# afriesen/rdis

Measured on AMD Instinct MI355X. Metric: subspace-solver iters/sec (all components), ladybug BA, higher is better.
Workload: dtype f64

## Files before the change

### rdis_amd/csrc/solver_pipe.hpp

```cpp
#pragma once
#include "solver_coop.hpp"

namespace rdis_hip {

constexpr int PIPE_NBUF = 32;
constexpr int PIPE_DEPTH = 3;
constexpr int PIPE_ENT = 512;
constexpr int PIPE_MAILS = 4;
constexpr int PIPE_THREADS = 256;
constexpr int PIPE_CTRL = 2;
constexpr int PIPE_LANES = PIPE_THREADS - 64 * PIPE_CTRL;
constexpr int PIPE_QUIT = 0x7FFFFFFF;
static_assert(PIPE_NBUF >= 5 * PIPE_DEPTH + 4 && (PIPE_NBUF & (PIPE_NBUF - 1)) == 0, "ring too short for the run-ahead");

struct PipeState {
    alignas(32) unsigned long long granule[2][PIPE_NBUF][PIPE_ENT][2];
    unsigned int abort_flag;
    unsigned int pad[15];
};
static_assert(sizeof(PipeState) <= sizeof(CoopState), "PipeState must fit the exchange state the host allocates");

struct alignas(16) PipeMail {
    int kind, flags;
    int e;
    int pad0;
    double a, b;
    double g_a, g_b, g_x, g_dx, g_ax, g_bx, g_cx;
    int g_need_first, g_known;
    double g_w, g_v, g_dw, g_dv, g_d, g_e, g_uu;
    int g_ph, pad1;
};
static_assert(sizeof(PipeMail) == 160, "mail layout");
constexpr int PIPE_RES = 4;
static_assert(PIPE_RES > PIPE_DEPTH, "result ring");
constexpr int PIPE_RECS = 8;
struct PipeShared {
    PipeMail mail[PIPE_MAILS];
    alignas(8) int seq;
    int verified;
    int pred_seq;
    int rec_slot[PIPE_RECS];
    double rec_val[PIPE_RECS];
    int cmd, cmd_delay;
    int res_slot[PIPE_RES];
    double res[PIPE_RES][3];
    int bar_done;
    int pub[PIPE_LANES / 64];
    int dead;
    int status, rolled_back, iter;
    int fin;
    long long nfeval, ngeval;
    double fret, finit;
    CgdMachine mach;
};
typedef __attribute__((address_space(3))) int lds_i32;
typedef __attribute__((address_space(3))) double lds_f64;
__device__ __forceinline__ int lds_int(const int& x) { return *(const volatile lds_i32*)&x; }
__device__ __forceinline__ void lds_set(int& x, int v) { *(volatile lds_i32*)&x = v; }
typedef __attribute__((address_space(3))) long long lds_i64;
__device__ __forceinline__ long long lds_int_pair(const int& x) { return *(const volatile lds_i64*)&x; }
__device__ __forceinline__ double lds_f64_get(const double& x) { return *(const volatile lds_f64*)&x; }
__device__ __forceinline__ void lds_f64_set(double& x, double v) { *(volatile lds_f64*)&x = v; }

struct PipeSync {
    PipeState* st;
    int tid, nwg, wg, nw;
    int poll_delay;
    int e;
    int rearmed;
    bool dead;
#ifdef RDIS_COOP_TIMING
    long long tm[COOP_TM];
#endif
    __device__ void tick(int slot, long long dt) {
#ifdef RDIS_COOP_TIMING
        tm[slot] += dt;
#endif
    }
    __device__ gu64* gran(int ex, int k, int w) const { return (gu64*)&st->granule[k >> 1][ex & (PIPE_NBUF - 1)][w][k & 1]; }
    __device__ u64x2 load_pair(int ex, int k, int w) const {
        u64x2 r;
        const gu64* p = gran(ex, k, w);
        asm volatile("global_load_dwordx4 %0, %1, off sc1" : "=v"(r) : "v"(p) : "memory");
        return r;
    }
    __device__ void store_pair(int ex, int k, int w, unsigned long long a, unsigned long long b) const {
        u64x2 t; t.x = a; t.y = b;
        gu64* p = gran(ex, k, w);
        asm volatile("global_store_dwordx4 %0, %1, off sc1" : : "v"(p), "v"(t) : "memory");
    }

    template <int N, int NMAX>
    __device__ void publish(int ex, double (&v)[N], int* pub) {
#pragma unroll
        for (int k = 0; k < N; ++k) v[k] = k < N - NMAX ? wave_sum(v[k]) : wave_max(v[k]);
        asm volatile("s_waitcnt vmcnt(0)" ::: "memory");
        if ((tid & 63) == 0) {
            const int ent = wg * nw + (tid >> 6) - PIPE_CTRL;
#pragma unroll
            for (int k = 0; k + 1 < N; k += 2) store_pair(ex, k, ent, GridSync::bits_of(v[k]), GridSync::bits_of(v[k + 1]));
            if constexpr (N & 1) GridSync::publish(gran(ex, N - 1, ent), v[N - 1]);
            lds_set(pub[(tid >> 6) - PIPE_CTRL], ex);
        }
    }

    template <int N, int NMAX>
    __device__ bool sweep(int ex, double (&v)[N], int delay, const int& cmd, int cmd_mine, const int* pub) {
        const int lane = tid & 63;
        const int nent = nwg * nw;
        double acc[N];
#pragma unroll
        for (int k = 0; k < N; ++k) acc[k] = 0.0;
        unsigned spins = 0;
        bool ok = !dead;
        const int per = (nent + 63) >> 6;
        constexpr int CH = 8;
        const long long tq0 = coop_clock();
        {
            bool waited = false;
            for (;;) {
                int lo = lds_int(pub[0]);
#pragma unroll
                for (int w = 1; w < PIPE_LANES / 64; ++w) { const int t = lds_int(pub[w]); lo = t < lo ? t : lo; }
                if (lo >= ex || dead) break;
                if (lds_int(cmd) != cmd_mine) return false;
                waited = true;
                if (++spins > COOP_SPIN_LIMIT) break;
                __builtin_amdgcn_s_sleep(1);
            }
            spins = 0;
            if (waited) { tick(26, coop_clock() - tq0); tick(27, 1); }
            if (waited) for (int d = 0; d < delay; d += 8) __builtin_amdgcn_s_sleep(8);
        }
        const long long tq1 = coop_clock();
        for (int j0 = 0; j0 < per && ok; j0 += CH) {
            unsigned long long val[CH][N];
#pragma unroll
            for (int j = 0; j < CH; ++j)
#pragma unroll
                for (int k = 0; k < N; ++k) val[j][k] = COOP_SENTINEL;
            for (;;) {
                tick(6, 1);
                constexpr int NP = N / 2;
                u64x2 pr[CH][NP > 0 ? NP : 1];
#pragma unroll
                for (int j = 0; j < CH; ++j) {
                    const int ww = lane + ((j0 + j) << 6);
                    const int wc = ww < nent ? ww : 0;
#pragma unroll
                    for (int k = 0; k + 1 < N; k += 2) {
                        pr[j][k / 2].x = val[j][k]; pr[j][k / 2].y = val[j][k + 1];
                        if (val[j][k] == COOP_SENTINEL || val[j][k + 1] == COOP_SENTINEL) pr[j][k / 2] = load_pair(ex, k, wc);
                    }
                    if constexpr (N & 1) {
                        if (val[j][N - 1] == COOP_SENTINEL)
                            val[j][N - 1] = __hip_atomic_load(gran(ex, N - 1, wc), __ATOMIC_RELAXED, __HIP_MEMORY_SCOPE_AGENT);
                    }
                }
                if constexpr (NP > 0) {
#pragma unroll
                    for (int j = 0; j < CH; ++j)
#pragma unroll
                        for (int q = 0; q < NP; ++q) asm volatile("" : "+v"(pr[j][q]));
                    asm volatile("s_waitcnt vmcnt(0)" ::: "memory");
#pragma unroll
                    for (int j = 0; j < CH; ++j)
#pragma unroll
                        for (int q = 0; q < NP; ++q) {
                            asm volatile("" : "+v"(pr[j][q]));
                            val[j][2 * q] = pr[j][q].x; val[j][2 * q + 1] = pr[j][q].y;
                        }
                }
                bool here = true;
#pragma unroll
                for (int j = 0; j < CH; ++j)
#pragma unroll
                    for (int k = 0; k < N; ++k) here = here && val[j][k] != COOP_SENTINEL;
                if (__all(here)) break;
                if (lds_int(cmd) != cmd_mine) return false;
                ++spins;
                if (spins > COOP_SPIN_LIMIT ||
                    ((spins & 255u) == 0u &&
                     __hip_atomic_load((gu32*)&st->abort_flag, __ATOMIC_RELAXED, __HIP_MEMORY_SCOPE_AGENT) != 0u)) {
                    if (lane == 0) __hip_atomic_store((gu32*)&st->abort_flag, 1u, __ATOMIC_RELAXED, __HIP_MEMORY_SCOPE_AGENT);
                    ok = false;
                    break;
                }
                __builtin_amdgcn_s_sleep(1);
            }
#pragma unroll
            for (int j = 0; j < CH; ++j) {
                if (lane + ((j0 + j) << 6) < nent) {
#pragma unroll
                    for (int k = 0; k < N; ++k) {
                        const double x = __longlong_as_double(val[j][k]);
                        if (k < N - NMAX) acc[k] += x; else acc[k] = fmax(acc[k], x);
                    }
                }
            }
        }
        if (!__all(ok)) dead = true;
        const long long tq2 = coop_clock();
#pragma unroll
        for (int k = 0; k < N; ++k) v[k] = k < N - NMAX ? wave_sum(acc[k]) : wave_max(acc[k]);
        tick(5, 1); tick(28, tq2 - tq1); tick(29, coop_clock() - tq2);
        return true;
    }
    __device__ void rearm_behind(int ex) {
        const int upto = ex - PIPE_DEPTH - 1;
        if ((tid & 63) < nw) {
            const int ent = wg * nw + (tid & 63);
            for (int x = rearmed + 1; x <= upto; ++x) {
#pragma unroll
                for (int k = 0; k < COOP_KP; k += 2) store_pair(x, k, ent, COOP_SENTINEL, COOP_SENTINEL);
            }
        }
        if (upto > rearmed) rearmed = upto;
    }

    __device__ void barrier(PipeShared& S) {
        double z[1] = {0.0};
        publish<1, 0>(e, z, S.pub);
        while (lds_int(S.bar_done) < e) __builtin_amdgcn_s_sleep(1);
        ++e;
        if (lds_int(S.dead) != 0) dead = true;
    }
};

struct PipeEnv {
    const ProblemView& P;
    const PlanView& L;
    const CoopArgs& A;
    PipeShared& S;
    int n, m, f0, c0;
    int gt, tid;
    PipeSync X;
    double* tr;
    int trn, lm_count;
    bool has_fac;
    int fid;
    int gpos[12];
    double base[12], dirv[12], lov[12], hiv[12];
    double ox, oy;
    VarState lv, wv;

    __device__ void trace(int tag, double a, double b, double c) {
        if (tr != nullptr && X.wg == 0 && tid == 0) {
            if (trn < L.trace_cap) { double* r = tr + 4ll * trn; r[0] = (double)tag; r[1] = a; r[2] = b; r[3] = c; }
            ++trn;
        }
    }

    template <bool SLOPE>
    __device__ void eval_line(double a, double& f, double& s) {
        double fj = 0.0, sj = 0.0;
        if (has_fac) {
            double v[12];
            {
#pragma clang fp contract(off)
#pragma unroll
                for (int k = 0; k < 12; ++k) {
                    const double t = a * dirv[k];
                    v[k] = clampd(base[k] + t, lov[k], hiv[k]);
                }
            }
            if constexpr (SLOPE) {
                double g[12];
                fj = ba_eval_grad(v, ox, oy, g);
                double acc = 0.0;
#pragma unroll
                for (int k = 0; k < 12; ++k) acc = __builtin_fma(g[k], dirv[k], acc);
                sj = acc;
            } else {
                fj = ba_eval(v, ox, oy);
            }
        }
        f = fj; s = sj;
    }
    __device__ void load_base(const double* vec) {
        if (has_fac) {
            const int c = P.cam[fid], q = P.pt[fid];
            const int* sl = A.slot_li + 12ll * gt;
#pragma unroll
            for (int k = 0; k < 12; ++k) {
                const int v = k < 9 ? c + k : q + (k - 9);
                const int li = sl[k];
                if (li >= 0) { base[k] = vec[li]; lov[k] = P.lo[v]; hiv[k] = P.hi[v]; }
                else { base[k] = P.x[v]; lov[k] = -__builtin_inf(); hiv[k] = __builtin_inf(); }
                dirv[k] = 0.0;
            }
        }
    }
    __device__ void var_init(VarState& V, int li) {
        V.li = li;
        V.p = V.xi = V.g = V.h = V.xinit = 0.0; V.lo = V.hi = 0.0;
        if (li >= 0) {
            const int vid = L.free_vid[f0 + li];
            V.p = L.xstart[f0 + li]; V.xinit = V.p;
            V.lo = P.lo[vid]; V.hi = P.hi[vid];
        }
    }
    __device__ void init_vectors() {
        var_init(lv, gt >= 0 ? A.lane_var[gt] : -1);
        var_init(wv, gt >= 0 ? A.wave_var[gt >> 6] : -1);
        load_base(L.xstart + f0);
    }
    __device__ void gradient_to_xi() {
        const long long tg0 = coop_clock();
        if (has_fac) {
            double v[12], g[12];
#pragma unroll
            for (int k = 0; k < 12; ++k) v[k] = clampd(base[k], lov[k], hiv[k]);
            ba_eval_grad(v, ox, oy, g);
#pragma unroll
            for (int k = 0; k < 12; ++k)
                if (gpos[k] >= 0) store_f64<true>(L.gfac + gpos[k], g[k]);
        }
        const long long tg1 = coop_clock();
        X.barrier(S);
        const long long tg2 = coop_clock();
        const int* vp = L.v2s_ptr + f0;
        if (lv.li >= 0) lv.xi = run_sum_ordered<true, 32>(L.gfac, vp[lv.li], vp[lv.li + 1]);
        if (wv.li >= 0) wv.xi = wave_sum(run_sum_strided<true>(L.gfac, vp[wv.li], vp[wv.li + 1], tid & 63));
        X.tick(3, tg1 - tg0); X.tick(18, tg2 - tg1); X.tick(30, coop_clock() - tg2); X.tick(31, 1);
    }
    __device__ void publish_xi() {
        if (lv.li >= 0) store_f64<true>(A.xi_glob + lv.li, lv.xi);
        if (wv.li >= 0 && (tid & 63) == 0) store_f64<true>(A.xi_glob + wv.li, wv.xi);
        X.barrier(S);
    }
    __device__ void cg_start() {
        { const double t = -lv.xi; lv.g = t; lv.h = t; lv.xi = t; }
        { const double t = -wv.xi; wv.g = t; wv.h = t; wv.xi = t; }
        publish_xi();
    }
    template <bool FROM_GH>
    __device__ void line_begin(double gam) {
        if (has_fac) {
            const int* sl = A.slot_li + 12ll * gt;
            int li[12];
#pragma unroll
            for (int k = 0; k < 12; ++k) li[k] = sl[k];
            double d[12];
            if constexpr (FROM_GH) {
                const double* gb = L.ws + 5ll * f0;
#pragma unroll
                for (int k = 0; k < 12; ++k) d[k] = load_f64<true>(gb + (li[k] >= 0 ? li[k] : 0));
                {
#pragma clang fp contract(off)
#pragma unroll
                    for (int k = 0; k < 12; ++k) d[k] = d[k] + gam * dirv[k];
                }
            } else {
#pragma unroll
                for (int k = 0; k < 12; ++k) d[k] = load_f64<true>(A.xi_glob + (li[k] >= 0 ? li[k] : 0));
            }
#pragma unroll
            for (int k = 0; k < 12; ++k) dirv[k] = li[k] >= 0 ? d[k] : 0.0;
        }
        if (L.vdump != nullptr && lm_count < L.dump_iters) {
            double* d = L.vdump + 2ll * L.dump_iters * f0 + 2ll * lm_count * n;
            if (lv.li >= 0) { d[lv.li] = lv.p; d[n + lv.li] = lv.xi; }
            if (wv.li >= 0 && (tid & 63) == 0) { d[wv.li] = wv.p; d[n + wv.li] = wv.xi; }
        }
        ++lm_count;
    }
    __device__ void line_end(double amin) {
#pragma clang fp contract(off)
        { const double t = lv.xi * amin; lv.xi = t; lv.p = lv.p + t; }
        { const double t = wv.xi * amin; wv.xi = t; wv.p = wv.p + t; }
        if (has_fac) {
#pragma unroll
            for (int k = 0; k < 12; ++k) { const double t = dirv[k] * amin; base[k] = base[k] + t; }
        }
    }
    __device__ void cg_reduce_publish(double fp) {
        {
            double* gb = L.ws + 5ll * f0;
            if (lv.li >= 0) store_f64<true>(gb + lv.li, -lv.xi);
            if (wv.li >= 0 && (tid & 63) == 0) store_f64<true>(gb + wv.li, -wv.xi);
        }
        double a = 0.0, b = 0.0, t = 0.0;
        {
#pragma clang fp contract(off)
            const double den = fmax(fabs(fp), 1.0);
            if (lv.li >= 0) {
                t = fabs(lv.xi) * fmax(fabs(lv.p), 1.0) / den;
                a = lv.g * lv.g;
                b = (lv.xi + lv.g) * lv.xi;
            }
            if (wv.li >= 0 && (tid & 63) == 0) {
                t = fmax(t, fabs(wv.xi) * fmax(fabs(wv.p), 1.0) / den);
                a = a + wv.g * wv.g;
                b = b + (wv.xi + wv.g) * wv.xi;
            }
        }
        double v[3] = {a, b, t};
        X.publish<3, 1>(X.e, v, S.pub);
        ++X.e;
    }
    __device__ void cg_update(double gam) {
#pragma clang fp contract(off)
        { const double gn = -lv.xi; const double hn = gn + gam * lv.h; lv.g = gn; lv.h = hn; lv.xi = hn; }
        { const double gn = -wv.xi; const double hn = gn + gam * wv.h; wv.g = gn; wv.h = hn; wv.xi = hn; }
    }
    __device__ void write_back(const VarState& V, bool restore, bool writer) {
        if (V.li >= 0 && writer) {
            const double xf = clampd(restore ? V.xinit : V.p, V.lo, V.hi);
            P.x[L.free_vid[f0 + V.li]] = xf;
            L.xout[f0 + V.li] = xf;
        }
    }
};

__device__ __forceinline__ int pipe_slot_owner(int i) {
    return (i == 0 || i == 2 || i == 3 || i == 18 || (i >= 9 && i <= 11) || i == 30 || i == 31) ? 2 : (i == 1 || (i >= 4 && i <= 6) || (i >= 26 && i <= 29)) ? 1 : 0;
}

__device__ __forceinline__ void pipe_post(PipeShared& S, int seq, int kind, int flags, int e, double a, double b, bool writer) {
    if (writer) {
        PipeMail* m = &S.mail[seq & (PIPE_MAILS - 1)];
        m->kind = kind; m->flags = flags; m->e = e; m->pad0 = 0; m->a = a; m->b = b;
        asm volatile("" ::: "memory");
        lds_set(S.seq, seq);
    }
}
__device__ __forceinline__ void pipe_post_predictor(PipeShared& S, int seq, const Predictor& G, bool writer) {
    if (writer) {
        PipeMail* m = &S.mail[seq & (PIPE_MAILS - 1)];
        m->g_ph = G.ph; m->g_need_first = G.need_first ? 1 : 0; m->g_known = G.known ? 1 : 0; m->pad1 = 0;
        m->g_a = G.a; m->g_b = G.b; m->g_x = G.x; m->g_dx = G.dx; m->g_ax = G.ax; m->g_bx = G.bx; m->g_cx = G.cx;
        m->g_w = G.w; m->g_v = G.v; m->g_dw = G.dw; m->g_dv = G.dv; m->g_d = G.d; m->g_e = G.e; m->g_uu = G.uu;
        asm volatile("" ::: "memory");
        lds_set(S.pred_seq, seq);
    }
}
__device__ __forceinline__ void pipe_command(PipeShared& S, int ex, int n, int delay, bool writer) {
    if (writer) { lds_set(S.cmd_delay, delay); lds_set(S.cmd, (ex << 2) | n); }
}
template <int N>
__device__ __forceinline__ void pipe_result(PipeShared& S, int ex, double (&v)[N], bool& dead) {
    while (lds_int(S.res_slot[ex & (PIPE_RES - 1)]) != ex) __builtin_amdgcn_s_sleep(1);
    asm volatile("" ::: "memory");
#pragma unroll
    for (int k = 0; k < N; ++k) v[k] = uniform(lds_f64_get(S.res[ex & (PIPE_RES - 1)][k]));
    if (lds_int(S.dead) != 0) dead = true;
}
__device__ __forceinline__ void pipe_ctrl_barrier(PipeSync& X, PipeShared& S, bool writer) {
    double z[1];
    pipe_command(S, X.e, 1, X.poll_delay, writer);
    pipe_result(S, X.e, z, X.dead);
    if (writer) lds_set(S.bar_done, X.e);
    ++X.e;
}

__device__ __forceinline__ void pipe_stepper(PipeEnv& E, PipeShared& S, int maxiters, double ftol) {
    CgdMachine& M = S.mach;
    const bool writer = E.tid == 0;
    if (writer) M.init(maxiters, ftol);
    int e_last = 0;
    bool chain_live = false;
    int next_free = 0;
    bool swapped = true;
    double r0 = 0.0, r1 = 0.0, r2 = 0.0;
    int seq = 0;
    bool guessed = false;
    double gval = 0.0;
    int ahead_slot = -1;
    double ahead0 = 0.0, ahead1 = 0.0;
    auto read_chain = [&]() {
        guessed = false; gval = 0.0; ahead_slot = -1; ahead0 = ahead1 = 0.0;
        if (chain_live) {
            const int z = e_last + 1;
            int rec = lds_int(S.rec_slot[z & (PIPE_RECS - 1)]);
            ahead_slot = lds_int(S.res_slot[z & (PIPE_RES - 1)]);
            ahead0 = lds_f64_get(S.res[z & (PIPE_RES - 1)][0]);
            ahead1 = lds_f64_get(S.res[z & (PIPE_RES - 1)][1]);
            while ((rec >> 1) != z) { __builtin_amdgcn_s_sleep(1); rec = lds_int(S.rec_slot[z & (PIPE_RECS - 1)]); }
            guessed = (rec & 1) != 0;
            gval = uniform(lds_f64_get(S.rec_val[z & (PIPE_RECS - 1)]));
        }
    };
    auto await_fd = [&](int e, bool hit) {
        double v[2];
        const long long tw0 = coop_clock();
        if (hit && __builtin_amdgcn_readfirstlane(ahead_slot) == e) {
            v[0] = uniform(ahead0); v[1] = uniform(ahead1);
            if (lds_int(S.dead) != 0) E.X.dead = true;
        } else {
            pipe_result(S, e, v, E.X.dead);
        }
        if (hit) { E.X.tick(20, coop_clock() - tw0); E.X.tick(16, 1); }
        else { E.X.tick(21, coop_clock() - tw0); E.X.tick(17, 1); }
        r0 = v[0]; r1 = v[1];
        e_last = e;
        chain_live = true;
        next_free = e_last + PIPE_DEPTH + 1;
    };
    for (;;) {
        long long ts0 = coop_clock();
        read_chain();
        bool stepped = false;
        if (__builtin_amdgcn_readfirstlane(lds_int(M.st)) == CgdMachine::S_DB_EVAL) {
            BrentHot s = M.brent();
            opaque(s.a); opaque(s.b); opaque(s.x); opaque(s.w); opaque(s.v); opaque(s.fx); opaque(s.fw); opaque(s.fv);
            opaque(s.dx); opaque(s.dw); opaque(s.dv); opaque(s.d); opaque(s.e); opaque(s.uu);
            HotPre P;
            CgdMachine::hot_pre(s, P);
            for (;;) {
                asm volatile("; PIPE_STEP_BEGIN");
                BrentHot n;
                double un;
                const bool take = CgdMachine::hot_post(s, P, r0, r1, n, un);
                if (__builtin_amdgcn_readfirstlane(take ? 1 : 0) == 0) break;
                s = n;
                if (E.X.dead) { stepped = true; break; }
                const bool hit = __builtin_amdgcn_readfirstlane((guessed && same_bits(un, gval)) ? 1 : 0) != 0;
                int e;
                if (hit) {
                    e = e_last + 1;
                    if (writer) lds_set(S.verified, e);
                } else {
                    e = next_free;
                    pipe_post(S, ++seq, REQ_EVAL, RF_SLOPE | RF_LINE, e, un, 0.0, writer);
                    Predictor G;
                    G.ph = Predictor::P_STOP; G.need_first = false; G.known = false; G.a = G.b = G.x = G.dx = 0.0; G.ax = G.bx = G.cx = 0.0;
                    G.w = G.v = G.dw = G.dv = G.d = G.e = G.uu = 0.0;
                    if (E.A.speculate) G.start_eval(s);
                    pipe_post_predictor(S, seq, G, writer);
                }
                asm volatile("; PIPE_STEP_END");
                const long long ts1 = coop_clock();
                E.X.tick(8, ts1 - ts0);
                E.X.e = e;
                if (!hit) pipe_command(S, e, 2, E.X.poll_delay, writer);
                CgdMachine::hot_pre(s, P);
                await_fd(e, hit);
                E.trace(TR_FD, un, r0, r1);
                E.X.tick(13, coop_clock() - ts1); E.X.tick(23, 1);
                ts0 = coop_clock();
                read_chain();
            }
            if (writer) M.set_brent(s);
        }
        asm volatile("; PIPE_GENERIC_BEGIN");
        Request nq;
        if (writer) {
            if (!stepped) {
                nq = M.next(r0, r1, r2);
                if (M.st == CgdMachine::S_BR_FC) swapped = M.ax == 1.0;
            } else {
                nq = CgdMachine::req(REQ_DONE);
            }
            if (E.X.dead) {
                nq = CgdMachine::req(REQ_DONE);
                M.reason = EXIT_SYNC_TIMEOUT; M.rolled_back = true; M.fret = M.finit;
            }
        }
        const int kind = __builtin_amdgcn_readfirstlane(nq.kind);
        const int flags = __builtin_amdgcn_readfirstlane(nq.flags);
        const bool slope = kind == REQ_EVAL && (flags & RF_SLOPE) != 0;
        const bool hit = __builtin_amdgcn_readfirstlane((slope && flags == (RF_SLOPE | RF_LINE) && guessed && same_bits(nq.a, gval)) ? 1 : 0) != 0;
        int e;
        if (hit) {
            e = e_last + 1;
            if (writer) lds_set(S.verified, e);
        } else {
            e = next_free;
            pipe_post(S, ++seq, kind, flags, e, nq.a, nq.b, writer);
            if (slope && writer) {
                Predictor G;
                G.ph = Predictor::P_STOP; G.need_first = false; G.known = false; G.a = G.b = G.x = G.dx = 0.0; G.ax = G.bx = G.cx = 0.0;
                G.w = G.v = G.dw = G.dv = G.d = G.e = G.uu = 0.0;
                if (E.A.speculate) G.start(M, swapped);
                pipe_post_predictor(S, seq, G, writer);
            }
        }
        if (E.tr != nullptr) {
            if ((flags & RF_TR_FIRST) && nq.tr_tag != TR_NONE) E.trace(nq.tr_tag, nq.tr_a, nq.tr_b, nq.tr_c);
            if (nq.pre_tag != TR_NONE) E.trace(nq.pre_tag, nq.pre_a, nq.pre_b, nq.pre_c);
            if (!(flags & RF_TR_FIRST) && nq.tr_tag != TR_NONE) E.trace(nq.tr_tag, nq.tr_a, nq.tr_b, nq.tr_c);
        }
        asm volatile("; PIPE_GENERIC_END");
        const long long ts1 = coop_clock();
        E.X.tick(8, ts1 - ts0);
        if (kind == REQ_DONE) break;
        E.X.e = e;
        chain_live = false;
        [[maybe_unused]] const int tkind = kind == REQ_GRAD ? 2 : !slope ? 0 : (flags & (RF_PRE_START | RF_PRE_UPDATE)) ? 3 : 1;
        switch (kind) {
        case REQ_EVAL:
            if (flags & RF_PRE_START) pipe_ctrl_barrier(E.X, S, writer);
            if (slope) {
                if (!hit) pipe_command(S, E.X.e, 2, E.X.poll_delay, writer);
                await_fd(E.X.e, hit);
                E.trace(TR_FD, nq.a, r0, r1);
            } else {
                double v[1];
                pipe_command(S, E.X.e, 1, E.X.poll_delay, writer);
                pipe_result(S, E.X.e, v, E.X.dead);
                r0 = v[0];
                next_free = E.X.e + 1;
                if (flags & RF_LINE) E.trace(TR_F, nq.a, r0, 0.0);
            }
            break;
        case REQ_GRAD:
            pipe_ctrl_barrier(E.X, S, writer);
            if (flags & RF_POST_REDUCE) {
                double v[3];
                pipe_command(S, E.X.e, 3, E.X.poll_delay, writer);
                pipe_result(S, E.X.e, v, E.X.dead);
                ++E.X.e;
                r1 = v[0]; r2 = v[1]; r0 = v[2];
            }
            next_free = E.X.e;
            break;
        default:
            break;
        }
        if (tkind == 0) { E.X.tick(12, coop_clock() - ts1); E.X.tick(22, 1); }
        else if (tkind == 1) { E.X.tick(13, coop_clock() - ts1); E.X.tick(23, 1); }
        else if (tkind == 2) { E.X.tick(14, coop_clock() - ts1); E.X.tick(24, 1); }
        else { E.X.tick(15, coop_clock() - ts1); E.X.tick(25, 1); }
    }
    if (writer) {
        lds_set(S.cmd, PIPE_QUIT);
        S.status = M.status(); S.rolled_back = M.rolled_back ? 1 : 0; S.iter = M.iter;
        S.nfeval = M.nfeval; S.ngeval = M.ngeval; S.fret = M.fret; S.finit = M.finit;
        asm volatile("" ::: "memory");
        lds_set(S.fin, 1);
    }
}

__device__ __forceinline__ void pipe_collector(PipeSync& X, PipeShared& S) {
    int mine = -1;
    int next = -1;
    const bool writer = (X.tid & 63) == 0;
    for (;;) {
        const int c = lds_int(S.cmd);
        int ex, n;
        if (c != mine) {
            if (c == PIPE_QUIT) break;
            mine = c;
            ex = c >> 2; n = c & 3;
        } else if (next >= 0) {
            ex = next; n = 2;
        } else {
            __builtin_amdgcn_s_sleep(1);
            continue;
        }
        next = -1;
        const int delay = lds_int(S.cmd_delay);
        double v[3] = {0.0, 0.0, 0.0};
        bool got;
        const long long t0 = coop_clock();
        if (n == 2) { double w[2]; got = X.sweep<2, 0>(ex, w, delay, S.cmd, mine, S.pub); v[0] = w[0]; v[1] = w[1]; }
        else if (n == 3) { got = X.sweep<3, 1>(ex, v, delay, S.cmd, mine, S.pub); }
        else { double w[1]; got = X.sweep<1, 0>(ex, w, delay, S.cmd, mine, S.pub); v[0] = w[0]; }
        if (!got) { X.tick(4, 1); continue; }
        X.tick(1, coop_clock() - t0);
        if (writer) {
            if (X.dead) lds_set(S.dead, 1);
            double* r = S.res[ex & (PIPE_RES - 1)];
            lds_f64_set(r[0], v[0]); lds_f64_set(r[1], v[1]); lds_f64_set(r[2], v[2]);
            lds_set(S.res_slot[ex & (PIPE_RES - 1)], ex);
        }
        asm volatile("s_waitcnt vmcnt(0)" ::: "memory");
        X.rearm_behind(ex);
        if (n == 2 && !X.dead) {
            const int z = ex + 1;
            for (;;) {
                const int rec = lds_int(S.rec_slot[z & (PIPE_RECS - 1)]);
                if ((rec >> 1) == z) { if (rec & 1) next = z; break; }
                if (lds_int(S.cmd) != mine) break;
                __builtin_amdgcn_s_sleep(1);
            }
        }
    }
}

__device__ __forceinline__ void pipe_record(PipeShared& S, int z, bool valid, double val, bool writer) {
    if (writer) {
        lds_f64_set(S.rec_val[z & (PIPE_RECS - 1)], val);
        lds_set(S.rec_slot[z & (PIPE_RECS - 1)], 2 * z + (valid ? 1 : 0));
    }
}
__device__ __forceinline__ void pipe_lanes(PipeEnv& E, PipeShared& S) {
    int seen = 0;
    const bool recorder = E.tid == 64 * PIPE_CTRL;
    for (;;) {
        int s;
        const long long tm0 = coop_clock();
        while ((s = lds_int(S.seq)) == seen) __builtin_amdgcn_s_sleep(1);
        E.X.tick(9, coop_clock() - tm0);
        seen = seen + 1;
        asm volatile("" ::: "memory");
        const PipeMail* m = &S.mail[seen & (PIPE_MAILS - 1)];
        const int kind = __builtin_amdgcn_readfirstlane(m->kind);
        const int flags = __builtin_amdgcn_readfirstlane(m->flags);
        E.X.e = __builtin_amdgcn_readfirstlane(m->e);
        const double qa = uniform(m->a);
        if (kind == REQ_DONE) break;
        if (kind == REQ_EVAL) {
            if (flags & RF_PRE_START) E.cg_start();
            if (flags & RF_PRE_UPDATE) E.cg_update(uniform(m->b));
            if (flags & RF_PRE_BEGIN) { if (flags & RF_PRE_UPDATE) E.line_begin<true>(uniform(m->b)); else E.line_begin<false>(0.0); }
            if (flags & RF_SLOPE) {
                const int e0 = E.X.e;
                {
                    double v[2];
                    const long long te0 = coop_clock();
                    E.eval_line<true>(qa, v[0], v[1]);
                    const long long te1 = coop_clock();
                    E.X.publish<2, 0>(e0, v, S.pub);
                    E.X.tick(0, te1 - te0); E.X.tick(2, coop_clock() - te1); E.X.tick(10, 1);

                }
                while (lds_int(S.pred_seq) < seen) __builtin_amdgcn_s_sleep(1);
                asm volatile("" ::: "memory");
                Predictor G;
                G.ph = __builtin_amdgcn_readfirstlane(m->g_ph);
                G.need_first = __builtin_amdgcn_readfirstlane(m->g_need_first) != 0;
                G.a = uniform(m->g_a); G.b = uniform(m->g_b); G.x = uniform(m->g_x); G.dx = uniform(m->g_dx);
                G.ax = uniform(m->g_ax); G.bx = uniform(m->g_bx); G.cx = uniform(m->g_cx);
                G.known = __builtin_amdgcn_readfirstlane(m->g_known) != 0;
                G.w = uniform(m->g_w); G.v = uniform(m->g_v); G.dw = uniform(m->g_dw); G.dv = uniform(m->g_dv);
                G.d = uniform(m->g_d); G.e = uniform(m->g_e); G.uu = uniform(m->g_uu);
                double cval = 0.0;
                bool cvalid = G.next(cval);
                int cz = e0 + 1;
                pipe_record(S, cz, cvalid, cval, recorder);
                for (;;) {
                    const long long sv = lds_int_pair(S.seq);
                    if (!cvalid || (int)sv != seen) break;
                    const int ver = (int)(sv >> 32);
                    if (cz > (ver > e0 ? ver : e0) + PIPE_DEPTH) { __builtin_amdgcn_s_sleep(1); continue; }
                    const double ca = cval;
                    const int z = cz;
                    cvalid = G.next(cval);
                    cz = z + 1;
                    pipe_record(S, cz, cvalid, cval, recorder);
                    double v[2];
                    const long long te0 = coop_clock();
                    E.eval_line<true>(ca, v[0], v[1]);
                    const long long te1 = coop_clock();
                    E.X.publish<2, 0>(z, v, S.pub);
                    E.X.tick(0, te1 - te0); E.X.tick(2, coop_clock() - te1); E.X.tick(11, 1);
                }
            } else {
                if (flags & RF_RESTORE) E.load_base(E.L.xstart + E.f0);
                double v[1], dummy;
                E.eval_line<false>((flags & RF_RESTORE) ? 0.0 : qa, v[0], dummy);
                E.X.publish<1, 0>(E.X.e, v, S.pub);
            }
        } else if (kind == REQ_GRAD) {
            if (flags & RF_PRE_LINE_END) E.line_end(qa);
            E.gradient_to_xi();
            if (flags & RF_POST_REDUCE) E.cg_reduce_publish(uniform(m->b));
        } else if (kind == REQ_LINE_END) {
            E.line_end(qa);
        }
    }
}

template <int THREADS>
__device__ __forceinline__ void pipe_solve(const ProblemView& P, const PlanView& L, const CoopArgs& A, int nwg, int wg,
                                           int maxiters, double ftol) {
    static_assert(THREADS == PIPE_THREADS, "stepper + collector + two lane waves");
    __shared__ PipeShared S;
    [[maybe_unused]] const long long tk0 = coop_clock();
    const int comp = A.comp;
    const int f0 = L.free_ptr[comp], c0 = L.fac_ptr[comp];
    const int n = L.free_ptr[comp + 1] - f0, m = L.fac_ptr[comp + 1] - c0;
    const int tid = (int)threadIdx.x;
    const int gt = tid < 64 * PIPE_CTRL ? -1 : wg * PIPE_LANES + tid - 64 * PIPE_CTRL;

    PipeEnv E{P, L, A, S, n, m, f0, c0, gt, tid,
              PipeSync{(PipeState*)A.st, tid, nwg, wg, PIPE_LANES / 64, A.poll_delay, 0, -1, false
#ifdef RDIS_COOP_TIMING
                       , {}
#endif
              },
              L.trace ? L.trace + 4ll * L.trace_cap * comp : nullptr, 0, 0,
              gt >= 0 && gt < m, 0, {}, {}, {}, {}, {}, 0.0, 0.0, {}, {}};
    if (tid == 0) { S.seq = 0; S.pred_seq = 0; S.cmd = -1; S.cmd_delay = 0; S.bar_done = -1; S.dead = 0; S.verified = -1; S.fin = 0; }
    if (tid < PIPE_RECS) S.rec_slot[tid] = -1;
    if (tid < PIPE_RES) S.res_slot[tid] = -1;
    if (tid < PIPE_LANES / 64) S.pub[tid] = -1;
    __syncthreads();
    const int role = __builtin_amdgcn_readfirstlane(tid >> 6);
    if (role == 0) pipe_stepper(E, S, maxiters, ftol);
    else if (role == 1) pipe_collector(E.X, S);
    else {
        if (E.has_fac) {
            E.fid = L.fac_id[c0 + gt];
            const double2 o = P.obs[E.fid];
            E.ox = o.x; E.oy = o.y;
            const int* sp = L.slot_pos + L.slot_base[c0 + gt];
#pragma unroll
            for (int k = 0; k < 12; ++k) E.gpos[k] = sp[k];
        }
        E.init_vectors();
        pipe_lanes(E, S);
        while (lds_int(S.fin) == 0) __builtin_amdgcn_s_sleep(1);
        const bool restore = S.rolled_back != 0;
        E.write_back(E.lv, restore, true);
        E.write_back(E.wv, restore, (tid & 63) == 0);
    }
    __syncthreads();
    if (wg == 0 && tid == 0) {
        L.fret[comp] = S.fret; L.delta[comp] = S.fret - S.finit; L.iters[comp] = S.iter;
        L.status[comp] = S.status; L.nfeval[comp] = S.nfeval; L.ngeval[comp] = S.ngeval;
        if (L.trace_n) L.trace_n[comp] = E.trn;
    }
#ifdef RDIS_COOP_TIMING
    if (wg == 0 && (tid & 63) == 0 && tid < 192 && A.timing) {
        if (tid == 0) E.X.tm[7] = coop_clock() - tk0;
        for (int i = 0; i < COOP_TM; ++i) if (pipe_slot_owner(i) == (tid >> 6)) A.timing[i] = E.X.tm[i];
    }
#endif
}

template <int THREADS>
__global__ void __launch_bounds__(THREADS)
cgd_pipe_kernel(ProblemView P, PlanView L, const CoopGroup* __restrict__ groups, const int* __restrict__ wg_group,
                int maxiters, double ftol) {
    const CoopGroup G = groups[wg_group[blockIdx.x]];
    pipe_solve<THREADS>(P, L, G.a, G.nwg, (int)blockIdx.x - G.wg0, maxiters, ftol);
}
template <int THREADS>
__global__ void __launch_bounds__(THREADS)
cgd_pipe_single_kernel(ProblemView P, PlanView L, CoopArgs A, int maxiters, double ftol) {
    pipe_solve<THREADS>(P, L, A, (int)gridDim.x, (int)blockIdx.x, maxiters, ftol);
}

__global__ void __launch_bounds__(256) pipe_arm_kernel(const CoopGroup* __restrict__ groups) {
    const CoopGroup G = groups[blockIdx.x / PIPE_NBUF];
    const int b = blockIdx.x % PIPE_NBUF;
    PipeState* st = (PipeState*)G.a.st;
    const int entries = G.nwg * (PIPE_LANES / 64);
    for (int t = threadIdx.x; t < COOP_KP * entries; t += blockDim.x) {
        const int k = t % COOP_KP, e = t / COOP_KP;
        st->granule[k >> 1][b][e][k & 1] = ~0ull;
    }
    if (b == 0 && threadIdx.x == 0) st->abort_flag = 0u;
}

inline int launch_pipe(hipStream_t stream, int kind, const ProblemView& P, const PlanView& V, const CoopGroup& first,
                       const CoopGroup* groups, const int* wg_group, int ngroups, int total_wg, int maxiters, double ftol) {
    if (kind != KIND_BA) return (int)hipErrorNotSupported;
    pipe_arm_kernel<<<ngroups * PIPE_NBUF, 256, 0, stream>>>(groups);
    hipError_t e0 = hipGetLastError();
    if (e0 != hipSuccess) return (int)e0;
    ProblemView p = P;
    PlanView v = V;
    int mi = maxiters;
    double ft = ftol;
    if (ngroups == 1) {
        CoopArgs a = first.a;
        void* args[] = {&p, &v, &a, &mi, &ft};
        return (int)hipLaunchCooperativeKernel((const void*)cgd_pipe_single_kernel<PIPE_THREADS>, dim3(total_wg), dim3(PIPE_THREADS), args, 0, stream);
    }
    const CoopGroup* gp = groups;
    const int* wp = wg_group;
    void* args[] = {&p, &v, &gp, &wp, &mi, &ft};
    return (int)hipLaunchCooperativeKernel((const void*)cgd_pipe_kernel<PIPE_THREADS>, dim3(total_wg), dim3(PIPE_THREADS), args, 0, stream);
}

inline int pipe_max_workgroups(int num_cus) {
    int per_cu = 0;
    if (hipOccupancyMaxActiveBlocksPerMultiprocessor(&per_cu, (const void*)cgd_pipe_kernel<PIPE_THREADS>, PIPE_THREADS, 0) != hipSuccess) return 0;
    if (per_cu > 1) per_cu -= 1;
    const long long cap = (long long)per_cu * num_cus;
    const long long lim = PIPE_ENT / (PIPE_LANES / 64);
    return (int)(cap > lim ? lim : cap);
}

}
```

Baseline: 10280.

## Replace gradient grid barrier with sentinel-flagged dataflow gather of factor gradients

Factor gradients are now published with relaxed atomic stores into slots pre-armed with a sentinel. Each variable's reducer spin-polls its own slots in chunks, sums them, then re-arms them with the sentinel. This removes the grid-wide barrier before the gradient reduction and the control-wave barrier in the REQ_GRAD path, so consumers wait only on the producers they need. The cost is polling traffic, an abort and timeout path, and an arm kernel that now also fills the gfac slots. It relies on ordering between the producer's stores and the re-arm for correctness.

```diff
diff --git a/rdis_amd/csrc/solver_pipe.hpp b/rdis_amd/csrc/solver_pipe.hpp
--- a/rdis_amd/csrc/solver_pipe.hpp
+++ b/rdis_amd/csrc/solver_pipe.hpp
@@ -305,6 +305,52 @@
         var_init(wv, gt >= 0 ? A.wave_var[gt >> 6] : -1);
         load_base(L.xstart + f0);
     }
+    template <int CH, int STRIDE>
+    __device__ bool gather_chunk(double* g, int k0, int e, unsigned long long (&val)[CH], unsigned& spins, long long& waited) {
+        const long long tw0 = coop_clock();
+#pragma unroll
+        for (int j = 0; j < CH; ++j) val[j] = k0 + STRIDE * j < e ? COOP_SENTINEL : 0ull;
+        bool ok = true;
+        for (;;) {
+#pragma unroll
+            for (int j = 0; j < CH; ++j) {
+                if (val[j] == COOP_SENTINEL) {
+                    const gu64* p = (const gu64*)(g + k0 + STRIDE * j);
+                    asm volatile("global_load_dwordx2 %0, %1, off sc1" : "+v"(val[j]) : "v"(p) : "memory");
+                }
+            }
+#pragma unroll
+            for (int j = 0; j < CH; ++j) asm volatile("" : "+v"(val[j]));
+            asm volatile("s_waitcnt vmcnt(0)" ::: "memory");
+#pragma unroll
+            for (int j = 0; j < CH; ++j) asm volatile("" : "+v"(val[j]));
+            bool here = true;
+#pragma unroll
+            for (int j = 0; j < CH; ++j) here = here && val[j] != COOP_SENTINEL;
+            if (__all(here)) break;
+            ++spins;
+            if (spins > COOP_SPIN_LIMIT ||
+                ((spins & 255u) == 0u &&
+                 __hip_atomic_load((gu32*)&X.st->abort_flag, __ATOMIC_RELAXED, __HIP_MEMORY_SCOPE_AGENT) != 0u)) {
+                if ((tid & 63) == 0) __hip_atomic_store((gu32*)&X.st->abort_flag, 1u, __ATOMIC_RELAXED, __HIP_MEMORY_SCOPE_AGENT);
+                ok = false;
+                break;
+            }
+            __builtin_amdgcn_s_sleep(1);
+        }
+        waited += coop_clock() - tw0;
+        if (ok) {
+#pragma unroll
+            for (int j = 0; j < CH; ++j)
+                if (k0 + STRIDE * j < e)
+                    __hip_atomic_store((gu64*)(g + k0 + STRIDE * j), COOP_SENTINEL, __ATOMIC_RELAXED, __HIP_MEMORY_SCOPE_AGENT);
+        }
+        return ok;
+    }
+    __device__ void gather_gave_up() {
+        X.dead = true;
+        if ((tid & 63) == 0) lds_set(S.dead, 1);
+    }
     __device__ void gradient_to_xi() {
         const long long tg0 = coop_clock();
         if (has_fac) {
@@ -314,15 +360,45 @@
             ba_eval_grad(v, ox, oy, g);
 #pragma unroll
             for (int k = 0; k < 12; ++k)
-                if (gpos[k] >= 0) store_f64<true>(L.gfac + gpos[k], g[k]);
+                if (gpos[k] >= 0)
+                    __hip_atomic_store((gu64*)(L.gfac + gpos[k]), GridSync::bits_of(g[k]), __ATOMIC_RELAXED, __HIP_MEMORY_SCOPE_AGENT);
         }
         const long long tg1 = coop_clock();
-        X.barrier(S);
-        const long long tg2 = coop_clock();
+        long long waited = 0;
+        unsigned spins = 0;
         const int* vp = L.v2s_ptr + f0;
-        if (lv.li >= 0) lv.xi = run_sum_ordered<true, 32>(L.gfac, vp[lv.li], vp[lv.li + 1]);
-        if (wv.li >= 0) wv.xi = wave_sum(run_sum_strided<true>(L.gfac, vp[wv.li], vp[wv.li + 1], tid & 63));
-        X.tick(3, tg1 - tg0); X.tick(18, tg2 - tg1); X.tick(30, coop_clock() - tg2); X.tick(31, 1);
+        {
+#pragma clang fp contract(off)
+            constexpr int CH = 16;
+            const int b = lv.li >= 0 ? vp[lv.li] : 0, e = lv.li >= 0 ? vp[lv.li + 1] : 0;
+            double s = 0.0;
+            for (int k0 = b; __any(k0 < e) && !X.dead; k0 += CH) {
+                unsigned long long val[CH];
+                if (!gather_chunk<CH, 1>(L.gfac, k0, e, val, spins, waited)) { gather_gave_up(); break; }
+#pragma unroll
+                for (int j = 0; j < CH; ++j) {
+                    const double t = __longlong_as_double(val[j]);
+                    if (k0 + j < e) s = (k0 + j == b) ? t : s + t;
+                }
+            }
+            if (lv.li >= 0) lv.xi = s;
+        }
+        if (wv.li >= 0) {
+#pragma clang fp contract(off)
+            constexpr int CH = 8;
+            const int lane = tid & 63;
+            const int b = vp[wv.li], e = vp[wv.li + 1];
+            double s = 0.0;
+            for (int k0 = b + lane; k0 - lane < e && !X.dead; k0 += 64 * CH) {
+                unsigned long long val[CH];
+                if (!gather_chunk<CH, 64>(L.gfac, k0, e, val, spins, waited)) { gather_gave_up(); break; }
+#pragma unroll
+                for (int j = 0; j < CH; ++j)
+                    if (k0 + 64 * j < e) s += __longlong_as_double(val[j]);
+            }
+            wv.xi = wave_sum(s);
+        }
+        X.tick(3, tg1 - tg0); X.tick(18, waited); X.tick(30, coop_clock() - tg1 - waited); X.tick(31, 1);
     }
     __device__ void publish_xi() {
         if (lv.li >= 0) store_f64<true>(A.xi_glob + lv.li, lv.xi);
@@ -605,7 +681,6 @@
             }
             break;
         case REQ_GRAD:
-            pipe_ctrl_barrier(E.X, S, writer);
             if (flags & RF_POST_REDUCE) {
                 double v[3];
                 pipe_command(S, E.X.e, 3, E.X.poll_delay, writer);
@@ -834,7 +909,8 @@
     pipe_solve<THREADS>(P, L, A, (int)gridDim.x, (int)blockIdx.x, maxiters, ftol);
 }
 
-__global__ void __launch_bounds__(256) pipe_arm_kernel(const CoopGroup* __restrict__ groups) {
+__global__ void __launch_bounds__(256) pipe_arm_kernel(const CoopGroup* __restrict__ groups, const int* __restrict__ free_ptr,
+                                                       const int* __restrict__ v2s_ptr, double* __restrict__ gfac) {
     const CoopGroup G = groups[blockIdx.x / PIPE_NBUF];
     const int b = blockIdx.x % PIPE_NBUF;
     PipeState* st = (PipeState*)G.a.st;
@@ -844,12 +920,17 @@
         st->granule[k >> 1][b][e][k & 1] = ~0ull;
     }
     if (b == 0 && threadIdx.x == 0) st->abort_flag = 0u;
+    const long long g0 = v2s_ptr[free_ptr[G.a.comp]], g1 = v2s_ptr[free_ptr[G.a.comp + 1]];
+    const long long per = (g1 - g0 + PIPE_NBUF - 1) / PIPE_NBUF;
+    const long long lo = g0 + b * per, hi = lo + per < g1 ? lo + per : g1;
+    unsigned long long* slots = reinterpret_cast<unsigned long long*>(gfac);
+    for (long long i = lo + threadIdx.x; i < hi; i += blockDim.x) slots[i] = COOP_SENTINEL;
 }
 
 inline int launch_pipe(hipStream_t stream, int kind, const ProblemView& P, const PlanView& V, const CoopGroup& first,
                        const CoopGroup* groups, const int* wg_group, int ngroups, int total_wg, int maxiters, double ftol) {
     if (kind != KIND_BA) return (int)hipErrorNotSupported;
-    pipe_arm_kernel<<<ngroups * PIPE_NBUF, 256, 0, stream>>>(groups);
+    pipe_arm_kernel<<<ngroups * PIPE_NBUF, 256, 0, stream>>>(groups, V.free_ptr, V.v2s_ptr, V.gfac);
     hipError_t e0 = hipGetLastError();
     if (e0 != hipSuccess) return (int)e0;
     ProblemView p = P;
```

Result: slower. 9813 (-4.5%).
